# arnaucube/babyjubjub-rs

Measured on AMD Instinct MI355X. Metric: BabyJubJub fixed-base scalar mults/sec, 1048576-item batch per GPU, higher is better.
Workload: dtype u32; 1 GPU; 1M fixed-base scalar mults (generator B8), BASELINE configs[1]; batch_per_gpu=1048576, global_batch=1048576, window_bits=28, table_bytes=154618823808, streams=2, kernel=bjj_k_mul_fixed_base_2x256, resident_batches=4, library_default_window_bits=23, parallelism=independent shards, one process per GPU, no data-path collective

## Files before the change

babyjubjub-rs_amd/csrc/curve.hpp:

```cpp
#pragma once
#include "fr.hpp"

namespace bjj {

struct Consts {
  Fr A, D;
  Fr F;
  Fr FINV_PLAIN;
  Fr FINV;
  Fr L_R1, L_R2;
  Fr DP, D2P, DPINV;
  Fr B8X, B8Y;
  Fr TS_G;
  Fr HALFQ;
  Fr ORDER, ORDER2, ORDER4;
  Fr L, L2, L4;
  Fr PCF[48];
  Fr PKP[60];
  Fr PSP[660];
  Fr PAL[25];
  Fr PM[36];
  Fr PCAB[30];
  Fr TSN[384];
  Fr TSH[448];
  unsigned char TSHASH[2048];
};
#define BJJ_CONSTS_INIT                                                                                                            \
  { BJJ_K_A, BJJ_K_D, BJJ_K_F, BJJ_K_FINV_PLAIN, BJJ_K_FINV, BJJ_K_L_R1, BJJ_K_L_R2, BJJ_K_DP, BJJ_K_D2P, BJJ_K_DPINV, BJJ_K_B8X,   \
    BJJ_K_B8Y, BJJ_K_TS_G, BJJ_K_HALFQ, BJJ_K_ORDER, BJJ_K_ORDER2, BJJ_K_ORDER4, BJJ_K_L, BJJ_K_L2, BJJ_K_L4, BJJ_K_POSEIDON_CF,   \
    BJJ_K_POSEIDON_KP, BJJ_K_POSEIDON_SP, BJJ_K_POSEIDON_AL, BJJ_K_POSEIDON_M, BJJ_K_POSEIDON_CAB, BJJ_K_TS_NEG, BJJ_K_TS_HALF,    \
    BJJ_K_TS_HASH }

struct Ext { Fr X, Y, Z, T; };
struct Niels { Fr ymx, ypx, t2d; };
struct PNiels { Fr ymx, ypx, t2d, z2; };
struct RefProj { Fr x, y, z; };

BJJ_HD Ext ext_identity() {
  Ext e; e.X = fr_zero(); e.Y = fr_one(); e.Z = fr_one(); e.T = fr_zero(); return e;
}


template <bool NEED_T = true>
BJJ_HD Ext ext_madd(const Ext& p, const Niels& q) {
  Fr a = fr_mul(fr_sub_lazy(p.Y, p.X), q.ymx);
  Fr b = fr_mul(fr_add_lazy(p.Y, p.X), q.ypx);
  Fr c = fr_mul(p.T, q.t2d);
  Fr d = fr_add_lazy(p.Z, p.Z);
  Fr e = fr_sub_lazy(b, a);
  Fr f = fr_sub(d, c);
  Fr g = fr_add_lazy(d, c);
  Fr h = fr_add_lazy(b, a);
  Ext r;
  r.X = fr_mul(e, f); r.Y = fr_mul(g, h); r.Z = fr_mul(f, g);
  if (NEED_T) r.T = fr_mul(e, h); else r.T = fr_zero();
  return r;
}
struct MaddState { Fr ym, yp, d, T; };
template <bool NEED_T = true>
BJJ_HD Ext ext_madd_state(const MaddState& s, const Niels& q, bool flip = false) {
  Fr a = fr_mul(s.ym, q.ymx);
  Fr b = fr_mul(s.yp, q.ypx);
  Fr c = fr_mul(s.T, q.t2d);
  Fr h = fr_add_lazy(b, a);
  Fr e;
#pragma unroll
  for (int i = 0; i < NL; i++) {
    const u32 x = flip ? a.v[i] : b.v[i];
    BJJ_ASSERT(h.v[i] - x <= fr_c4limb(i));
    e.v[i] = (x << 1) + fr_c4limb(i) - h.v[i];
  }
  Fr f = fr_sub(s.d, c);
  Fr g = fr_add_lazy(s.d, c);
  Ext r;
  r.X = fr_mul(e, f); r.Y = fr_mul(g, h); r.Z = fr_mul(f, g);
  if (NEED_T) r.T = fr_mul(e, h); else r.T = fr_zero();
  return r;
}
BJJ_HD MaddState ext_madd_forms(const Ext& p) {
  MaddState s;
  s.ym = fr_sub_lazy(p.Y, p.X); s.yp = fr_add_lazy(p.Y, p.X); s.d = fr_add_lazy(p.Z, p.Z); s.T = p.T;
  return s;
}
BJJ_HD MaddState niels_tform_state(const Niels& e0, bool neg, bool neg_t) {
  MaddState s;
  const Fr ymx = fr_select(neg, e0.ypx, e0.ymx), ypx = fr_select(neg, e0.ymx, e0.ypx);
  s.ym = fr_add_lazy(ymx, ymx);
  s.yp = fr_add_lazy(ypx, ypx);
  s.d = fr_add(fr_add(fr_one(), fr_one()), fr_add(fr_one(), fr_one()));
  s.T = fr_select(neg_t, fr_sub_lazy(fr_zero(), e0.t2d), e0.t2d);
  return s;
}
BJJ_HD Ext ext_add_pn(const Ext& p, const PNiels& q, bool need_t = true) {
  Fr a = fr_mul(fr_sub_lazy(p.Y, p.X), q.ymx);
  Fr b = fr_mul(fr_add_lazy(p.Y, p.X), q.ypx);
  Fr c = fr_mul(p.T, q.t2d);
  Fr d = fr_mul(p.Z, q.z2);
  Fr e = fr_sub_lazy(b, a);
  Fr f = fr_sub(d, c);
  Fr g = fr_add_lazy(d, c);
  Fr h = fr_add_lazy(b, a);
  Ext r;
  r.X = fr_mul(e, f); r.Y = fr_mul(g, h); r.Z = fr_mul(f, g);
  r.T = fr_zero();
  if (need_t) r.T = fr_mul(e, h);
  return r;
}
template <bool NEED_T>
BJJ_HD Ext ext_dbl(const Ext& p) {
  Fr a = fr_sqr(p.X), b = fr_sqr(p.Y), zz = fr_sqr(p.Z);
  Fr h = fr_add_lazy(a, b);
  Fr s = fr_sqr(fr_add_lazy(p.X, p.Y));
  Fr e = fr_sub8_of_lazy(s, h);
  Fr g = fr_sub_lazy(b, a);
  Fr f = fr_sub(fr_add_lazy(fr_add_lazy(zz, zz), a), b);
  Ext r;
  r.X = fr_mul(e, f); r.Y = fr_mul(g, h); r.Z = fr_mul(f, g);
  if (NEED_T) r.T = fr_mul(e, h); else r.T = fr_zero();
  return r;
}
BJJ_HD PNiels ext_to_pniels(const Ext& p, const Consts& K) {
  PNiels n;
  n.ymx = fr_sub(p.Y, p.X); n.ypx = fr_add(p.Y, p.X);
  n.t2d = fr_mul(p.T, K.D2P); n.z2 = fr_dbl(p.Z);
  return n;
}
BJJ_HD PNiels pniels_cneg(const PNiels& n, bool neg) {
  PNiels r;
  r.ymx = fr_select(neg, n.ypx, n.ymx);
  r.ypx = fr_select(neg, n.ymx, n.ypx);
  r.t2d = fr_select(neg, fr_sub_lazy(fr_zero(), n.t2d), n.t2d);
  r.z2 = n.z2;
  return r;
}
BJJ_HD Ext ext_from_ref_affine(const Fr& x, const Fr& y, const Consts& K) {
  Ext e;
  e.X = fr_mul(x, K.F); e.Y = y; e.Z = fr_one(); e.T = fr_mul(e.X, y);
  return e;
}
BJJ_HD bool ref_on_curve(const Fr& x, const Fr& y, const Consts& K) {
  Fr x2 = fr_sqr(x), y2 = fr_sqr(y);
  Fr lhs = fr_add(fr_mul(K.A, x2), y2);
  Fr rhs = fr_add(fr_one(), fr_mul(K.D, fr_mul(x2, y2)));
  return fr_eq(lhs, rhs);
}

BJJ_HD RefProj ref_add(const RefProj& p, const RefProj& q, const Consts& K) {
  Fr a = fr_mul(p.z, q.z);
  Fr b = fr_sqr(a);
  Fr c = fr_mul(p.x, q.x);
  Fr d = fr_mul(p.y, q.y);
  Fr e = fr_mul(fr_mul(K.D, c), d);
  Fr f = fr_sub(b, e);
  Fr g = fr_add(b, e);
  Fr aux = fr_mul(fr_add(p.x, p.y), fr_add(q.x, q.y));
  aux = fr_sub(fr_sub(aux, c), d);
  Fr x3 = fr_mul(fr_mul(a, f), aux);
  Fr dac = fr_sub(d, fr_mul(K.A, c));
  Fr y3 = fr_mul(fr_mul(a, g), dac);
  RefProj r; r.x = x3; r.y = y3; r.z = fr_mul(f, g);
  return r;
}

BJJ_HD void scalar_mod_order(const u32 w[8], u32 out[8], const Consts& K) {
  Fr s = fr_from_words(w);
  s = fr_cond_sub_kr(s, K.ORDER4.v);
  s = fr_cond_sub_kr(s, K.ORDER2.v);
  s = fr_cond_sub_kr(s, K.ORDER.v);
  fr_to_words(s, out);
}
BJJ_HD Fr plain_mod_l(const Fr& v, const Consts& K) {
  Fr s = fr_cond_sub_kr(v, K.L4.v);
  s = fr_cond_sub_kr(s, K.L2.v);
  s = fr_cond_sub_kr(s, K.L.v);
  return s;
}
BJJ_HD u32 scalar_window(const u32 w[8], int j, int W) {
  const int bit = j * W, wi = bit >> 5, sh = bit & 31;
  if (wi >= 8) return 0;
  u64 two = (u64)w[wi] | ((u64)(wi + 1 < 8 ? w[wi + 1] : 0u) << 32);
  return (u32)(two >> sh) & ((1u << W) - 1u);
}

}
```

babyjubjub-rs_amd/csrc/fr.hpp:

```cpp
#pragma once
#include <stdint.h>

#if defined(__HIPCC__)
#define BJJ_HD __host__ __device__ __forceinline__
#define BJJ_HD_NOINLINE static __host__ __device__ __noinline__
#else
#define BJJ_HD inline
#define BJJ_HD_NOINLINE
#endif

#if defined(BJJ_DEBUG_BOUNDS) && !defined(__HIP_DEVICE_COMPILE__)
#include <assert.h>
#define BJJ_ASSERT(x) assert(x)
#else
#define BJJ_ASSERT(x) ((void)0)
#endif

namespace bjj {

typedef uint32_t u32;
typedef uint64_t u64;

constexpr int NL = 9;
constexpr u32 MASK29 = 0x1fffffffu;

struct Fr { u32 v[NL]; };

#define BJJ_N0 0x10000001u
#define BJJ_N1 0x1f0fac9fu
#define BJJ_N2 0x0e5c2450u
#define BJJ_N3 0x07d090f3u
#define BJJ_N4 0x1585d283u
#define BJJ_N5 0x02db40c0u
#define BJJ_N6 0x00a6e141u
#define BJJ_N7 0x0e5c2634u
#define BJJ_N8 0x0030644eu
#define BJJ_NINV29 0x0fffffffu

BJJ_HD u32 fr_modlimb(int i) {
  constexpr u32 N[NL] = {BJJ_N0, BJJ_N1, BJJ_N2, BJJ_N3, BJJ_N4, BJJ_N5, BJJ_N6, BJJ_N7, BJJ_N8};
  return N[i];
}

BJJ_HD u32 fr_c4limb(int i) {
  constexpr u32 C[NL] = {0x4u + 0x20000000u, 0x1c3eb27eu + 0x1fffffffu, 0x19709143u + 0x1fffffffu,
                         0x1f4243cdu + 0x1fffffffu, 0x16174a0cu + 0x1fffffffu, 0x0b6d0302u + 0x1fffffffu,
                         0x029b8504u + 0x1fffffffu, 0x197098d0u + 0x1fffffffu, 0x00c19139u - 1u};
  return C[i];
}
BJJ_HD u32 fr_c8limb(int i) {
  constexpr u32 C[NL] = {0x8u + 0x20000000u, 0x187d64fcu + 0x1fffffffu, 0x12e12287u + 0x1fffffffu,
                         0x1e84879bu + 0x1fffffffu, 0x0c2e9419u + 0x1fffffffu, 0x16da0605u + 0x1fffffffu,
                         0x05370a08u + 0x1fffffffu, 0x12e131a0u + 0x1fffffffu, 0x01832273u - 1u};
  return C[i];
}

BJJ_HD Fr fr_zero() { Fr r; for (int i = 0; i < NL; i++) r.v[i] = 0; return r; }

BJJ_HD void fr_carry(Fr& a) {
#pragma unroll
  for (int i = 0; i < NL - 1; i++) {
    a.v[i + 1] += a.v[i] >> 29;
    a.v[i] &= MASK29;
  }
}

BJJ_HD Fr fr_add(const Fr& a, const Fr& b) {
  Fr r;
#pragma unroll
  for (int i = 0; i < NL; i++) r.v[i] = a.v[i] + b.v[i];
  fr_carry(r);
  return r;
}
BJJ_HD Fr fr_sub(const Fr& a, const Fr& b) {
  Fr r;
  BJJ_ASSERT(b.v[8] <= fr_c4limb(8));
#pragma unroll
  for (int i = 0; i < NL; i++) r.v[i] = a.v[i] + fr_c4limb(i) - b.v[i];
  fr_carry(r);
  return r;
}
BJJ_HD Fr fr_sub8(const Fr& a, const Fr& b) {
  Fr r;
  BJJ_ASSERT(b.v[8] <= fr_c8limb(8));
#pragma unroll
  for (int i = 0; i < NL; i++) r.v[i] = a.v[i] + fr_c8limb(i) - b.v[i];
  fr_carry(r);
  return r;
}
BJJ_HD Fr fr_add_lazy(const Fr& a, const Fr& b) {
  Fr r;
#pragma unroll
  for (int i = 0; i < NL; i++) r.v[i] = a.v[i] + b.v[i];
  return r;
}
BJJ_HD Fr fr_sub_lazy(const Fr& a, const Fr& b) {
  Fr r;
  BJJ_ASSERT(b.v[8] <= fr_c4limb(8));
#pragma unroll
  for (int i = 0; i < NL; i++) { BJJ_ASSERT(b.v[i] <= fr_c4limb(i)); r.v[i] = a.v[i] + fr_c4limb(i) - b.v[i]; }
  return r;
}
BJJ_HD u32 fr_k8limb(int i) {
  constexpr u32 C[NL] = {0x8u + 0x40000000u, 0x187d64fcu + 0x3ffffffeu, 0x12e12287u + 0x3ffffffeu,
                         0x1e84879bu + 0x3ffffffeu, 0x0c2e9419u + 0x3ffffffeu, 0x16da0605u + 0x3ffffffeu,
                         0x05370a08u + 0x3ffffffeu, 0x12e131a0u + 0x3ffffffeu, 0x01832273u - 2u};
  return C[i];
}
BJJ_HD Fr fr_sub8_of_lazy(const Fr& a, const Fr& b) {
  Fr r;
#pragma unroll
  for (int i = 0; i < NL; i++) { BJJ_ASSERT(b.v[i] <= fr_k8limb(i)); r.v[i] = a.v[i] + fr_k8limb(i) - b.v[i]; }
  fr_carry(r);
  return r;
}
BJJ_HD Fr fr_neg(const Fr& a) { return fr_sub(fr_zero(), a); }
BJJ_HD Fr fr_dbl(const Fr& a) { return fr_add(a, a); }

BJJ_HD Fr fr_select(bool c, const Fr& a, const Fr& b) {
  Fr r;
#pragma unroll
  for (int i = 0; i < NL; i++) r.v[i] = c ? a.v[i] : b.v[i];
  return r;
}

#if defined(BJJ_DEBUG_BOUNDS) && !defined(__HIP_DEVICE_COMPILE__)
inline void fr_check_mul_operands(const Fr& a, const Fr& b) {
  for (int k = 0; k < 2 * NL - 1; k++) {
    unsigned __int128 col = 0;
    for (int i = 0; i < NL; i++) { int j = k - i; if (j >= 0 && j < NL) col += (unsigned __int128)a.v[i] * b.v[j]; }
    col += (unsigned __int128)9 * 0x1fffffffULL * 0x1fffffffULL + ((unsigned __int128)1 << 36);
    assert((col >> 64) == 0);
  }
  unsigned __int128 ah = (((unsigned __int128)a.v[8] << 29) + a.v[7]) + 1;
  unsigned __int128 bh = (((unsigned __int128)b.v[8] << 29) + b.v[7]) + 1;
  const unsigned __int128 lim = (((unsigned __int128)0x30644e72e131ULL << 64) | 0xa029b85045b68181ULL) >> 1;
  assert(ah * bh <= lim);
}
#define BJJ_CHECK_MUL(a, b) fr_check_mul_operands(a, b)
#else
#define BJJ_CHECK_MUL(a, b) ((void)0)
#endif

#define BJJ_MAD(acc, x, y) acc += (u64)(x) * (y)
#define BJJ_MAD_K(acc, x, k) acc += (u64)(x) * (k)

#if defined(__HIP_DEVICE_COMPILE__) && !defined(BJJ_NO_ASM_COLUMNS)
#include "fr_mul_columns.inc"
#endif

BJJ_HD Fr fr_mul(const Fr& a, const Fr& b) {
  BJJ_CHECK_MUL(a, b);
#if defined(__HIP_DEVICE_COMPILE__) && !defined(BJJ_NO_ASM_COLUMNS)
  return fr_mul_columns(a, b);
#endif
  u32 m[NL];
  Fr r;
  u64 acc = 0;
#pragma unroll
  for (int k = 0; k < NL; k++) {
#pragma unroll
    for (int i = 0; i <= k; i++) BJJ_MAD(acc, a.v[i], b.v[k - i]);
#pragma unroll
    for (int i = 0; i < k; i++) BJJ_MAD_K(acc, m[i], fr_modlimb(k - i));
    m[k] = ((u32)acc * BJJ_NINV29) & MASK29;
    BJJ_MAD_K(acc, m[k], BJJ_N0);
    acc >>= 29;
  }
#pragma unroll
  for (int k = NL; k < 2 * NL - 1; k++) {
#pragma unroll
    for (int i = k - (NL - 1); i < NL; i++) BJJ_MAD(acc, a.v[i], b.v[k - i]);
#pragma unroll
    for (int i = k - (NL - 1); i < NL; i++) BJJ_MAD_K(acc, m[i], fr_modlimb(k - i));
    r.v[k - NL] = (u32)acc & MASK29;
    acc >>= 29;
  }
  r.v[NL - 1] = (u32)acc;
  return r;
}

BJJ_HD Fr fr_sqr(const Fr& a) {
  BJJ_CHECK_MUL(a, a);
#if defined(__HIP_DEVICE_COMPILE__) && !defined(BJJ_NO_ASM_COLUMNS)
  return fr_sqr_columns(a);
#endif
  u32 m[NL], a2[NL];
#pragma unroll
  for (int i = 0; i < NL; i++) a2[i] = a.v[i] << 1;
  Fr r;
  u64 acc = 0;
#pragma unroll
  for (int k = 0; k < NL; k++) {
#pragma unroll
    for (int i = 0; 2 * i < k; i++) BJJ_MAD(acc, a2[i], a.v[k - i]);
    if ((k & 1) == 0) BJJ_MAD(acc, a.v[k / 2], a.v[k / 2]);
#pragma unroll
    for (int i = 0; i < k; i++) BJJ_MAD_K(acc, m[i], fr_modlimb(k - i));
    m[k] = ((u32)acc * BJJ_NINV29) & MASK29;
    BJJ_MAD_K(acc, m[k], BJJ_N0);
    acc >>= 29;
  }
#pragma unroll
  for (int k = NL; k < 2 * NL - 1; k++) {
#pragma unroll
    for (int i = k - (NL - 1); 2 * i < k; i++) BJJ_MAD(acc, a2[i], a.v[k - i]);
    if ((k & 1) == 0) BJJ_MAD(acc, a.v[k / 2], a.v[k / 2]);
#pragma unroll
    for (int i = k - (NL - 1); i < NL; i++) BJJ_MAD_K(acc, m[i], fr_modlimb(k - i));
    r.v[k - NL] = (u32)acc & MASK29;
    acc >>= 29;
  }
  r.v[NL - 1] = (u32)acc;
  return r;
}

BJJ_HD Fr fr_reduce_weak(const Fr& x) {
  const u32 q = x.v[8] / 3171407u;
  Fr r;
  int64_t c = 0;
#pragma unroll
  for (int i = 0; i < NL; i++) {
    c += (int64_t)x.v[i] - (int64_t)((u64)q * fr_modlimb(i));
    r.v[i] = (i < NL - 1) ? ((u32)c & MASK29) : (u32)c;
    c >>= 29;
  }
  return r;
}

BJJ_HD Fr fr_one() {
  Fr r = {{0x0fffff57u, 0x1ea70ab4u, 0x052c068bu, 0x17504f49u, 0x0aa8075bu, 0x1d4240ceu, 0x11d54c07u, 0x052ac7a8u, 0x000dc836u}};
  return r;
}
BJJ_HD Fr fr_r2() {
  Fr r = {{0x05b69bd4u, 0x06170a5au, 0x020cddceu, 0x1db6310bu, 0x0e54d0ffu, 0x1cf855e3u, 0x1c15e103u, 0x07d09161u, 0x000a054au}};
  return r;
}
BJJ_HD Fr fr_one_plain() { Fr r = fr_zero(); r.v[0] = 1; return r; }

BJJ_HD Fr fr_from_words(const u32 w[8]) {
  Fr r;
  r.v[0] = w[0] & MASK29;
#pragma unroll
  for (int i = 1; i < 8; i++) {
    const int bit = 29 * i, wi = bit >> 5, sh = bit & 31;
    u64 two = (u64)w[wi] | ((u64)(wi + 1 < 8 ? w[wi + 1] : 0u) << 32);
    r.v[i] = (u32)(two >> sh) & MASK29;
  }
  r.v[8] = w[7] >> 8;
  return r;
}
BJJ_HD void fr_to_words(const Fr& a, u32 w[8]) {
#pragma unroll
  for (int j = 0; j < 8; j++) {
    const int bit = 32 * j, li = bit / 29, sh = bit - 29 * li;
    u64 acc = (u64)a.v[li] >> sh;
    int have = 29 - sh;
    acc |= (u64)a.v[li + 1] << have;
    have += 29;
    if (have < 32 && li + 2 < NL) acc |= (u64)a.v[li + 2] << have;
    w[j] = (u32)acc;
  }
}

BJJ_HD Fr fr_cond_sub_kr(const Fr& x, const u32 kr[NL]) {
  Fr d;
  u32 borrow = 0;
#pragma unroll
  for (int i = 0; i < NL; i++) {
    u32 t = x.v[i] - kr[i] - borrow;
    borrow = t >> 31;
    d.v[i] = (i < NL - 1) ? (t & MASK29) : t;
  }
  return fr_select(borrow != 0, x, d);
}
BJJ_HD Fr fr_canon(const Fr& x) {
  constexpr u32 R8[NL] = {0x8u, 0x187d64fcu, 0x12e12287u, 0x1e84879bu, 0x0c2e9419u, 0x16da0605u, 0x05370a08u, 0x12e131a0u, 0x01832273u};
  constexpr u32 R4[NL] = {0x4u, 0x1c3eb27eu, 0x19709143u, 0x1f4243cdu, 0x16174a0cu, 0x0b6d0302u, 0x029b8504u, 0x197098d0u, 0x00c19139u};
  constexpr u32 R2[NL] = {0x2u, 0x1e1f593fu, 0x1cb848a1u, 0x0fa121e6u, 0x0b0ba506u, 0x05b68181u, 0x014dc282u, 0x1cb84c68u, 0x0060c89cu};
  constexpr u32 R1[NL] = {BJJ_N0, BJJ_N1, BJJ_N2, BJJ_N3, BJJ_N4, BJJ_N5, BJJ_N6, BJJ_N7, BJJ_N8};
  Fr t = fr_cond_sub_kr(x, R8);
  t = fr_cond_sub_kr(t, R4);
  t = fr_cond_sub_kr(t, R2);
  t = fr_cond_sub_kr(t, R1);
  return t;
}
BJJ_HD bool fr_is_zero_canon(const Fr& a) {
  u32 o = 0;
#pragma unroll
  for (int i = 0; i < NL; i++) o |= a.v[i];
  return o == 0;
}
BJJ_HD bool fr_is_zero(const Fr& a) { return fr_is_zero_canon(fr_canon(a)); }
BJJ_HD bool fr_eq(const Fr& a, const Fr& b) { return fr_is_zero(fr_sub(a, b)); }

BJJ_HD Fr fr_to_mont_words(const u32 w[8]) { return fr_mul(fr_from_words(w), fr_r2()); }
BJJ_HD void fr_from_mont_words(const Fr& a, u32 w[8]) {
  constexpr u32 R1[NL] = {BJJ_N0, BJJ_N1, BJJ_N2, BJJ_N3, BJJ_N4, BJJ_N5, BJJ_N6, BJJ_N7, BJJ_N8};
  Fr t = fr_mul(a, fr_one_plain());
  t = fr_cond_sub_kr(t, R1);
  fr_to_words(t, w);
}

BJJ_HD_NOINLINE Fr fr_inv_fermat(const Fr& a) {
  const u32 E[8] = {0xefffffffu, 0x43e1f593u, 0x79b97091u, 0x2833e848u, 0x8181585du, 0xb85045b6u, 0xe131a029u, 0x30644e72u};
  Fr x = a;
  for (int bit = 252; bit >= 0; bit--) {
    x = fr_sqr(x);
    if ((E[bit >> 5] >> (bit & 31)) & 1) x = fr_mul(x, a);
  }
  return x;
}

BJJ_HD_NOINLINE Fr fr_inv_gcd(const Fr& x) {
  constexpr u32 R32[NL] = {0x20u, 0x01f593f0u, 0x0b848a1fu, 0x1a121e6eu, 0x10ba5067u, 0x1b681815u, 0x14dc2822u, 0x0b84c680u, 0x060c89ceu};
  constexpr u32 R16[NL] = {0x10u, 0x10fac9f8u, 0x05c2450fu, 0x1d090f37u, 0x185d2833u, 0x0db40c0au, 0x0a6e1411u, 0x05c26340u, 0x030644e7u};
  constexpr u32 R8[NL] = {0x8u, 0x187d64fcu, 0x12e12287u, 0x1e84879bu, 0x0c2e9419u, 0x16da0605u, 0x05370a08u, 0x12e131a0u, 0x01832273u};
  constexpr u32 R4[NL] = {0x4u, 0x1c3eb27eu, 0x19709143u, 0x1f4243cdu, 0x16174a0cu, 0x0b6d0302u, 0x029b8504u, 0x197098d0u, 0x00c19139u};
  constexpr u32 R2c[NL] = {0x2u, 0x1e1f593fu, 0x1cb848a1u, 0x0fa121e6u, 0x0b0ba506u, 0x05b68181u, 0x014dc282u, 0x1cb84c68u, 0x0060c89cu};
  constexpr u32 R1[NL] = {BJJ_N0, BJJ_N1, BJJ_N2, BJJ_N3, BJJ_N4, BJJ_N5, BJJ_N6, BJJ_N7, BJJ_N8};
  Fr a = fr_canon(x);
  Fr b, u = fr_r2(), v = fr_zero();
#pragma unroll
  for (int i = 0; i < NL; i++) b.v[i] = fr_modlimb(i);
#pragma unroll 1
  for (int outer = 0; outer < 18; outer++) {
    u32 ah = 0, al = 0, all_ = 0, bh = 0, bl = 0, bll = 0;
    int top = 0;
#pragma unroll
    for (int i = NL - 1; i >= 2; i--) {
      const bool hit = (top == 0) && ((a.v[i] | b.v[i]) != 0);
      ah = hit ? a.v[i] : ah; al = hit ? a.v[i - 1] : al; all_ = hit ? a.v[i - 2] : all_;
      bh = hit ? b.v[i] : bh; bl = hit ? b.v[i - 1] : bl; bll = hit ? b.v[i - 2] : bll;
      top = hit ? i : top;
    }
    const int L = (top == 0) ? 0 : 32 - __builtin_clz(ah | bh);
    const bool big = 29 * top + L > 60, l2 = L >= 2;
    const int sh = l2 ? L - 2 : 0;
    const u64 ha = ((u64)ah << 29) | al, hb = ((u64)bh << 29) | bl;
    const u64 ta_s = ha >> sh, tb_s = hb >> sh;
    const u64 ta_l = (ha << 1) | (all_ >> 28), tb_l = (hb << 1) | (bll >> 28);
    const u64 ta = l2 ? ta_s : ta_l, tb = l2 ? tb_s : tb_l;
    const u64 xa_big = (ta << 29) | a.v[0], xb_big = (tb << 29) | b.v[0];
    const u64 xa_small = ((u64)a.v[2] << 58) | ((u64)a.v[1] << 29) | a.v[0];
    const u64 xb_small = ((u64)b.v[2] << 58) | ((u64)b.v[1] << 29) | b.v[0];
    u64 xa = big ? xa_big : xa_small, xb = big ? xb_big : xb_small;
    int32_t f0 = 1, g0 = 0, f1 = 0, g1 = 1;
#pragma unroll 1
    for (int i = 0; i < 29; i++) {
      const bool odd = (xa & 1) != 0;
// ... 144 lines not shown
```

babyjubjub-rs_amd/csrc/k_fixed.hip:

```cpp
#include "k_common.hpp"

#ifndef BJJ_K1_BLOCK
#define BJJ_K1_BLOCK BJJ_EPI_BLOCK
#endif
#ifndef BJJ_K1_MIN_BLOCKS
#define BJJ_K1_MIN_BLOCKS 1
#endif
#ifndef BJJ_K1_NBUF
#define BJJ_K1_NBUF 2
#endif
#ifndef BJJ_K1_INV_CORE
#define BJJ_K1_INV_CORE INV_K1
#endif
#ifndef BJJ_K1_PIPE_ITEM
#define BJJ_K1_PIPE_ITEM 1
#endif
#ifndef BJJ_K1_PIPE_RECORD
#define BJJ_K1_PIPE_RECORD 0
#endif
#ifndef BJJ_K1_EARLY_RECORD
#define BJJ_K1_EARLY_RECORD 0
#endif
#ifndef BJJ_K1_LATE_SCALAR
#define BJJ_K1_LATE_SCALAR 1
#endif
#ifndef BJJ_K1_FOLD_LIFT
#define BJJ_K1_FOLD_LIFT 1
#endif
#ifndef BJJ_K1_WEAK_MOD_L
#define BJJ_K1_WEAK_MOD_L 1
#endif
#ifndef BJJ_K1_SLOT_STRIP
#define BJJ_K1_SLOT_STRIP 1
#endif
#ifndef BJJ_K1_SIGN_CARRY
#define BJJ_K1_SIGN_CARRY 1
#endif
#ifndef BJJ_K1_REG_RECORDS
#define BJJ_K1_REG_RECORDS 1
#endif
#ifndef BJJ_K1_UNIFORM_STAGE
#define BJJ_K1_UNIFORM_STAGE 1
#endif
#ifndef BJJ_K1_ALIGN_DIGITS
#define BJJ_K1_ALIGN_DIGITS 1
#endif
#define K1_SIGN_CARRY (BJJ_K1_SIGN_CARRY && BJJ_K1_FOLD_LIFT)

__global__ void __launch_bounds__(64) bjj_k_fixed_window_bases(u32* bases, int W, int nwin) {
  const int j = blockIdx.x * blockDim.x + threadIdx.x;
  if (j >= nwin) return;
  store_niels(bases + (size_t)j * NIELS_WORDS, fixed_table_entry(1u, j, W, c_K));
}
__global__ void __launch_bounds__(BJJ_BLOCK) bjj_k_build_fixed_table(u32* table, const u32* __restrict__ bases, int W, int nwin,
                                                                 u32 chain) {
  const size_t stride = fixed_stride(W);
  const size_t cpw = (stride + chain - 1) / chain;
  const size_t t = (size_t)blockIdx.x * blockDim.x + threadIdx.x;
  if (t >= cpw * (size_t)nwin) return;
  const int j = (int)(t / cpw);
  const size_t k0 = (t % cpw) * chain;
  const u32 cnt = (u32)(stride - k0 < chain ? stride - k0 : chain);
  fixed_table_chain(table, load_niels(bases + (size_t)j * NIELS_WORDS), (size_t)j * stride + k0, (u32)k0, cnt, W, c_K);
}
__global__ void __launch_bounds__(BJJ_BLOCK) bjj_k_check_fixed_table(const u32* __restrict__ table, const u32* __restrict__ bases,
                                                                 int W, int nwin, unsigned long long* bad) {
  const size_t stride = fixed_stride(W);
  const size_t total = stride * (size_t)nwin, nthreads = (size_t)gridDim.x * blockDim.x;
  unsigned long long mine = 0;
#pragma unroll 1
  for (size_t e = (size_t)blockIdx.x * blockDim.x + threadIdx.x; e < total; e += nthreads)
    mine += (unsigned long long)fixed_table_check_slot(table, bases, (int)(e / stride), (u32)(e % stride), W, nwin, c_K);
  if (mine) atomicAdd(bad, mine);
}


struct K1Item {
  DigitStream ds;
  bool neg0, neg1;
};
__device__ __forceinline__ u32 k1_limb(u32 lo, u32 hi, int sh) { return ((lo >> sh) | (hi << (32 - sh))) & MASK29; }
__device__ __forceinline__ Fr k1_scalar_limbs(const U4 (&v)[2]) {
  Fr s;
  s.v[0] = v[0].x & MASK29;
  s.v[1] = k1_limb(v[0].x, v[0].y, 29); s.v[2] = k1_limb(v[0].y, v[0].z, 26); s.v[3] = k1_limb(v[0].z, v[0].w, 23);
  s.v[4] = k1_limb(v[0].w, v[1].x, 20); s.v[5] = k1_limb(v[1].x, v[1].y, 17); s.v[6] = k1_limb(v[1].y, v[1].z, 14);
  s.v[7] = k1_limb(v[1].z, v[1].w, 11);
  s.v[8] = v[1].w >> 8;
  return s;
}
__device__ __forceinline__ size_t k1_digit_next(DigitStream& d, bool& neg) {
  if (!BJJ_K1_ALIGN_DIGITS) return digit_next(d, neg);
  const u32 u = (d.w[0] & d.mask) + d.carry;
  neg = u > d.half;
  d.carry = neg ? 1u : 0u;
  const u32 dig = neg ? (d.mask + 1u) - u : u;
  const size_t slot = d.base + dig;
  d.base += d.stride;
#pragma unroll
  for (int i = 0; i < 7; i++) d.w[i] = __builtin_amdgcn_alignbit(d.w[i + 1], d.w[i], (u32)d.W);
  d.w[7] >>= d.W;
  return slot;
}
template <class G>
__device__ __forceinline__ K1Item k1_item_begin(const G& g, int W, const U4 (&scalar)[2]) {
  u32 sc[8];
  Fr s = scalar_mod_l_weak_limbs(k1_scalar_limbs(scalar), scalar[1].w >> 24, c_K);
  if (!BJJ_K1_WEAK_MOD_L) s = fr_cond_sub_kr(s, c_K.L.v);
  fr_to_words(s, sc);
  K1Item it;
  it.ds = digit_stream(sc, W);
  typename G::Pending p;
  g.issue(k1_digit_next(it.ds, it.neg0), p, 0);
  g.issue(k1_digit_next(it.ds, it.neg1), p, 1);
  return it;
}
#if BJJ_K1_FOLD_LIFT
typedef MaddState K1Acc;
template <bool NEED_T = true>
__device__ __forceinline__ Ext k1_madd(const K1Acc& s, const Niels& q, bool flip = false) {
  return ext_madd_state<NEED_T>(s, q, K1_SIGN_CARRY && flip);
}
__device__ __forceinline__ K1Acc k1_forms(const Ext& p) { return ext_madd_forms(p); }
#else
typedef Ext K1Acc;
template <bool NEED_T = true>
__device__ __forceinline__ Ext k1_madd(const K1Acc& s, const Niels& q, bool = false) { return ext_madd<NEED_T>(s, q); }
__device__ __forceinline__ K1Acc k1_forms(const Ext& p) { return p; }
#endif
__device__ __forceinline__ Niels k1_entry(const Niels& e, bool neg) { return K1_SIGN_CARRY ? e : niels_cneg_lazy(e, neg); }
template <class G, class MID>
__device__ __forceinline__ void k1_item_windows(const G& g, int nwin, K1Item& it, K1Acc& acc, Niels& cur, const MID& mid) {
  typename G::Pending p;
  bool neg, last = false;
#if K1_SIGN_CARRY
  acc = niels_tform_state(g.finish(p, 0), it.neg0 != it.neg1, it.neg0 != it.neg1);
  BJJ_SCHED_FENCE();
  cur = g.finish(p, 1);
  last = it.neg1;
#elif BJJ_K1_FOLD_LIFT
  const Niels e0 = g.finish(p, 0);
  const Fr ymx0 = fr_select(it.neg0, e0.ypx, e0.ymx), ypx0 = fr_select(it.neg0, e0.ymx, e0.ypx);
  acc.ym = fr_add_lazy(ymx0, ymx0);
  acc.yp = fr_add_lazy(ypx0, ypx0);
  acc.d = fr_add(fr_add(fr_one(), fr_one()), fr_add(fr_one(), fr_one()));
  acc.T = e0.t2d;
  BJJ_SCHED_FENCE();
  const Niels e1 = g.finish(p, 1);
  cur = niels_cneg_lazy(e1, it.neg1);
  cur.t2d = fr_select(it.neg0 != it.neg1, fr_sub_lazy(fr_zero(), e1.t2d), e1.t2d);
#else
  const Niels n0 = niels_cneg_lazy(g.finish(p, 0), it.neg0);
  acc.X = fr_reduce_weak(fr_sub(n0.ypx, n0.ymx));
  acc.Y = fr_add(n0.ypx, n0.ymx);
  acc.Z = fr_add(fr_one(), fr_one()); acc.T = fr_add(n0.t2d, fr_zero());
  BJJ_SCHED_FENCE();
  cur = niels_cneg_lazy(g.finish(p, 1), it.neg1);
#endif
  mid();
#pragma unroll 1
  for (int j = 1; j + 1 < nwin; j++) {
    g.issue(k1_digit_next(it.ds, neg), p, (j + 1) & 1);
    acc = k1_forms(k1_madd(acc, cur, neg != last));
    if (K1_SIGN_CARRY) last = neg;
    BJJ_SCHED_FENCE();
    cur = k1_entry(g.finish(p, (j + 1) & 1), neg);
  }
}
struct K1Stash { U4 x[2], y[2], z[2], p[2]; };
__device__ __forceinline__ void k1_words(U4 (&v)[2], const Fr& f) {
  const u32* a = f.v;
  v[0] = U4{a[0] | (a[1] << 29), (a[1] >> 3) | (a[2] << 26), (a[2] >> 6) | (a[3] << 23), (a[3] >> 9) | (a[4] << 20)};
  v[1] = U4{(a[4] >> 12) | (a[5] << 17), (a[5] >> 15) | (a[6] << 14), (a[6] >> 18) | (a[7] << 11), (a[7] >> 21) | (a[8] << 8)};
}
__device__ __forceinline__ void k1_stash_words(U4 (&v)[2], const Fr& f) {
  if (BJJ_K1_REG_RECORDS) { k1_words(v, f); return; }
  u32 w[8];
  fr_to_words(f, w);
  v[0] = U4{w[0], w[1], w[2], w[3]}; v[1] = U4{w[4], w[5], w[6], w[7]};
}
__device__ __forceinline__ void k1_stash_pack(K1Stash& s, const Ext& p, Fr& run) {
  k1_stash_words(s.x, p.X); k1_stash_words(s.y, p.Y); k1_stash_words(s.z, p.Z); k1_stash_words(s.p, run);
  run = fr_mul(run, p.Z);
}
__device__ __forceinline__ void k1_stash_store(const K1Stash& s, uint8_t* xy_item, u32* scr_item) {
  U4 *q = (U4*)xy_item, *r = (U4*)scr_item;
  q[0] = s.x[0]; q[1] = s.x[1]; q[2] = s.y[0]; q[3] = s.y[1];
  r[0] = s.z[0]; r[1] = s.z[1]; r[2] = s.p[0]; r[3] = s.p[1];
}
struct K1Record {
  U4 z[2], p[2], x[2], y[2];
};
__device__ __forceinline__ void k1_record_load(K1Record& r, const uint8_t* xy_item, const u32* scr_item) {
  const U4 *s = (const U4*)scr_item, *q = (const U4*)xy_item;
  r.z[0] = s[0]; r.z[1] = s[1]; r.p[0] = s[2]; r.p[1] = s[3];
  r.x[0] = q[0]; r.x[1] = q[1]; r.y[0] = q[2]; r.y[1] = q[3];
}
__device__ __forceinline__ Fr k1_record_fr(const U4 (&v)[2]) {
  if (BJJ_K1_REG_RECORDS) return k1_scalar_limbs(v);
  const u32 w[8] = {v[0].x, v[0].y, v[0].z, v[0].w, v[1].x, v[1].y, v[1].z, v[1].w};
  return fr_from_words(w);
}
template <unsigned FORM>
__device__ __forceinline__ void k1_record_finish(Fr& inv, uint8_t* out_item, const K1Record& r) {
  constexpr u32 R1[NL] = {BJJ_N0, BJJ_N1, BJJ_N2, BJJ_N3, BJJ_N4, BJJ_N5, BJJ_N6, BJJ_N7, BJJ_N8};
  const Fr Z = k1_record_fr(r.z), P = k1_record_fr(r.p), X = k1_record_fr(r.x), Y = k1_record_fr(r.y);
  Fr zinv = fr_mul(inv, P);
  inv = fr_mul(inv, Z);
  Fr c2 = fr_mul(zinv, c_K.FINV);
  Fr x = fr_cond_sub_kr(fr_mul(X, c2), R1);
  Fr y = fr_cond_sub_kr(fr_mul(Y, zinv), R1);
  if (BJJ_K1_REG_RECORDS) {
    U4 *const o = (U4*)out_item, v[2];
    if (FORM & EPI_COMPRESS) {
      k1_words(v, y);
      if (plain_gt_halfq(x, c_K)) v[1].w |= 0x80000000u;
      o[0] = v[0]; o[1] = v[1];
    } else {
      k1_words(v, x); o[0] = v[0]; o[1] = v[1];
      k1_words(v, y); o[2] = v[0]; o[3] = v[1];
    }
    return;
  }
  u32 w[8];
  if (FORM & EPI_COMPRESS) {
    fr_to_words(y, w);
    if (plain_gt_halfq(x, c_K)) w[7] |= 0x80000000u;
    store_w8(out_item, w);
  } else {
    fr_to_words(x, w); store_w8(out_item, w);
    fr_to_words(y, w); store_w8(out_item + 32, w);
  }
}
template <int BLOCK, unsigned FORM>
__device__ __forceinline__ void k1_epilogue_run(Fr run, size_t n, size_t tid, size_t nthreads, uint8_t* out, const uint8_t* stash,
                                                const u32* scratch, u32* lds) {
  constexpr size_t OUT_BYTES = (FORM & EPI_COMPRESS) ? 32 : 64;
  const size_t cnt = tid < n ? (n - tid + nthreads - 1) / nthreads : 0;
  K1Record cur;
  if (BJJ_K1_EARLY_RECORD && cnt) {
    asm volatile("s_waitcnt vmcnt(0)" ::: "memory");
    const size_t i = tid + (cnt - 1) * nthreads;
    k1_record_load(cur, stash + i * 64, scratch + i * 16);
  }
  Fr inv = fr_mul(block_invert<BLOCK, BJJ_K1_INV_CORE>(run, lds), fr_one_plain());
  if (!cnt) return;
  if (!BJJ_K1_EARLY_RECORD) {
    const size_t i = tid + (cnt - 1) * nthreads;
    k1_record_load(cur, stash + i * 64, scratch + i * 16);
  }
#pragma unroll 1
  for (size_t m = cnt; m-- > 0;) {
    const size_t i = tid + m * nthreads;
    if (BJJ_K1_PIPE_RECORD) {
      K1Record nxt = cur;
      if (m) k1_record_load(nxt, stash + (i - nthreads) * 64, scratch + (i - nthreads) * 16);
      k1_record_finish<FORM>(inv, out + i * OUT_BYTES, cur);
      cur = nxt;
    } else {
      k1_record_finish<FORM>(inv, out + i * OUT_BYTES, cur);
      if (m) k1_record_load(cur, stash + (i - nthreads) * 64, scratch + (i - nthreads) * 16);
    }
  }
}

template <int BLOCK, int NBUF, unsigned FORM = EPI_AFFINE, bool AHEAD = false>
__device__ __forceinline__ void mul_fixed_base_body(const u32* __restrict__ table, int W, int nwin, const uint8_t* __restrict__ scalars,
                                                    size_t n, uint8_t* __restrict__ out, u32* __restrict__ scratch,
                                                    uint8_t* __restrict__ xy = nullptr) {
  __shared__ u32 lds[NL * 64];
  constexpr bool STRIP = AHEAD && BJJ_K1_PIPE_ITEM && BJJ_K1_SLOT_STRIP;
  constexpr int WAVE_WORDS = NBUF * FB_STAGE_WORDS + (STRIP ? FB_STRIP_WORDS : 0);
  __shared__ __attribute__((aligned(16))) u32 stage[(BLOCK / 64) * WAVE_WORDS];
  const size_t tid = (size_t)blockIdx.x * blockDim.x + threadIdx.x;
  const size_t nthreads = (size_t)gridDim.x * blockDim.x;
  const int lane = threadIdx.x & 63;
  const int wave = AHEAD && BJJ_K1_UNIFORM_STAGE ? __builtin_amdgcn_readfirstlane((int)(threadIdx.x >> 6)) : (int)(threadIdx.x >> 6);
  const GatherCoopLds<NBUF, STRIP> fb = {table, stage + wave * WAVE_WORDS, lane};
  uint8_t* const stash = (FORM & EPI_COMPRESS) ? xy : out;
  Fr run = fr_one();
  if (AHEAD && BJJ_K1_PIPE_ITEM) {
    static_assert(!AHEAD || NBUF >= 2, "both gathers of the next item are issued at once");
    size_t i = tid;
    if (i - lane < n) {
      const U4* const sc4 = (const U4*)scalars;
      U4 raw[2] = {sc4[2 * (i < n ? i : n - 1)], sc4[2 * (i < n ? i : n - 1) + 1]};
      K1Item it = k1_item_begin(fb, W, raw);
      K1Stash held = {};
      bool pending = false;
      size_t iheld = 0;
#pragma unroll 1
      for (;;) {
        const size_t inext = i + nthreads, iload = inext < n ? inext : n - 1;
        const bool more = inext - lane < n;
        if (!BJJ_K1_LATE_SCALAR && more) { raw[0] = sc4[2 * iload]; raw[1] = sc4[2 * iload + 1]; }
        K1Acc acc;
        Niels cur;
        k1_item_windows(fb, nwin, it, acc, cur, [&]() {
          if (!BJJ_K1_LATE_SCALAR) return;
          if (pending) k1_stash_store(held, stash + iheld * 64, scratch + iheld * 16);
          if (more) { raw[0] = sc4[2 * iload]; raw[1] = sc4[2 * iload + 1]; }
        });
        if (more) it = k1_item_begin(fb, W, raw);
        BJJ_SCHED_FENCE();
        const Ext p = k1_madd<false>(acc, cur);
        pending = BJJ_K1_LATE_SCALAR && more;
        if (pending) { k1_stash_pack(held, p, run); iheld = i; }
        else if (i < n) {
          if (BJJ_K1_REG_RECORDS) { k1_stash_pack(held, p, run); k1_stash_store(held, stash + i * 64, scratch + i * 16); }
          else epilogue_stash(p, run, stash + i * 64, scratch + i * 16);
        }
        if (!more) break;
        i = inext;
      }
    }
  } else {
#pragma unroll 1
    for (size_t i = tid; i - lane < n; i += nthreads) {
      const bool valid = i < n;
      u32 sc[8];
      load_w8(scalars + (valid ? i : n - 1) * 32, sc);
      Ext p = fixed_base_mul(fb, W, nwin, sc, c_K);
      if (valid) epilogue_stash(p, run, stash + i * 64, scratch + i * 16);
    }
  }
  if (AHEAD && (BJJ_K1_REG_RECORDS || BJJ_K1_PIPE_RECORD || BJJ_K1_EARLY_RECORD))
    k1_epilogue_run<BLOCK, FORM>(run, n, tid, nthreads, out, stash, scratch, lds);
  else
    epilogue_run<BLOCK, FORM, BJJ_K1_INV_CORE>(run, n, tid, nthreads, out, scratch, lds, xy);
}
__global__ void __launch_bounds__(BJJ_K1_BLOCK, BJJ_K1_MIN_BLOCKS) bjj_k_mul_fixed_base(const u32* __restrict__ table, int W, int nwin,
                                                                  const uint8_t* __restrict__ scalars, size_t n,
                                                                  uint8_t* __restrict__ out, u32* __restrict__ scratch) {
  mul_fixed_base_body<BJJ_K1_BLOCK, BJJ_K1_NBUF>(table, W, nwin, scalars, n, out, scratch);
}
template <unsigned FORM>
__device__ __forceinline__ void mul_fixed_base_scan_body(const u32* __restrict__ table, int W, const uint8_t* __restrict__ scalars, size_t n,
                                                         uint8_t* __restrict__ out, u32* __restrict__ scratch, uint8_t* __restrict__ xy, int nwin) {
  __shared__ u32 lds[NL * 64];
  const size_t tid = (size_t)blockIdx.x * blockDim.x + threadIdx.x;
  const size_t nthreads = (size_t)gridDim.x * blockDim.x;
  const GatherScan fb = {table, (u32)fixed_stride(W)};
  Fr run = fr_one();
#pragma unroll 1
  for (size_t i = tid; i < n; i += nthreads) {
    u32 sc[8];
    load_w8(scalars + i * 32, sc);
    Ext p = fixed_base_mul(fb, W, nwin, sc, c_K);
    epilogue_stash(p, run, ((FORM & EPI_COMPRESS) ? xy : out) + i * 64, scratch + i * 16);
  }
  epilogue_run<BJJ_EPI_BLOCK, FORM, BJJ_K1_INV_CORE>(run, n, tid, nthreads, out, scratch, lds, xy);
}
__global__ void __launch_bounds__(BJJ_EPI_BLOCK, 1) bjj_k_mul_fixed_base_scan(const u32* __restrict__ table, int W, int nwin,
                                                                        const uint8_t* __restrict__ scalars, size_t n,
                                                                        uint8_t* __restrict__ out, u32* __restrict__ scratch) {
  mul_fixed_base_scan_body<EPI_AFFINE>(table, W, scalars, n, out, scratch, nullptr, nwin);
}
__global__ void __launch_bounds__(256, 2) bjj_k_mul_fixed_base_2x256(const u32* __restrict__ table, int W, int nwin,
                                                                    const uint8_t* __restrict__ scalars, size_t n,
                                                                    uint8_t* __restrict__ out, u32* __restrict__ scratch) {
  mul_fixed_base_body<256, 2, EPI_AFFINE, true>(table, W, nwin, scalars, n, out, scratch);
}
__global__ void __launch_bounds__(BJJ_K1_BLOCK, BJJ_K1_MIN_BLOCKS) bjj_k_mul_fixed_base_c32(const u32* __restrict__ table, int W, int nwin,
                                                                      const uint8_t* __restrict__ scalars, size_t n,
                                                                      uint8_t* __restrict__ out32, u32* __restrict__ scratch,
                                                                      uint8_t* __restrict__ xy) {
  mul_fixed_base_body<BJJ_K1_BLOCK, BJJ_K1_NBUF, EPI_COMPRESS>(table, W, nwin, scalars, n, out32, scratch, xy);
}
__global__ void __launch_bounds__(256, 2) bjj_k_mul_fixed_base_2x256_c32(const u32* __restrict__ table, int W, int nwin,
                                                                        const uint8_t* __restrict__ scalars, size_t n,
                                                                        uint8_t* __restrict__ out32, u32* __restrict__ scratch,
                                                                        uint8_t* __restrict__ xy) {
  mul_fixed_base_body<256, 2, EPI_COMPRESS, true>(table, W, nwin, scalars, n, out32, scratch, xy);
}
__global__ void __launch_bounds__(BJJ_EPI_BLOCK, 1) bjj_k_mul_fixed_base_scan_c32(const u32* __restrict__ table, int W, int nwin,
                                                                            const uint8_t* __restrict__ scalars, size_t n,
                                                                            uint8_t* __restrict__ out32, u32* __restrict__ scratch,
                                                                            uint8_t* __restrict__ xy) {
  mul_fixed_base_scan_body<EPI_COMPRESS>(table, W, scalars, n, out32, scratch, xy, nwin);
}

namespace bjjk {
int fixed_base_lanes_per_cu(int variant) {
  return variant ? lanes_for_both(bjj_k_mul_fixed_base_2x256, bjj_k_mul_fixed_base_2x256_c32, 256)
                 : lanes_for_both(bjj_k_mul_fixed_base, bjj_k_mul_fixed_base_c32, BJJ_K1_BLOCK);
}
hipError_t fill_fixed_table(hipStream_t st, u32* table, const u32* bases, int W, int nwin) {
  const size_t entries = fixed_stride(W) * (size_t)nwin;
  size_t chain = entries >> 18;
  chain = chain < 4 ? 4 : (chain > 256 ? 256 : chain);
  const size_t chains = ((fixed_stride(W) + chain - 1) / chain) * (size_t)nwin;
  BJJ_LAUNCH(bjj_k_build_fixed_table, dim3((unsigned)((chains + BJJ_BLOCK - 1) / BJJ_BLOCK)), dim3(BJJ_BLOCK), 0, st,
                     table, bases, W, nwin, (u32)chain);
  return hipGetLastError();
}
hipError_t build_fixed_table(hipStream_t st, u32* table, u32* bases, int W, int nwin) {
  BJJ_LAUNCH(bjj_k_fixed_window_bases, dim3((nwin + 63) / 64), dim3(64), 0, st, bases, W, nwin);
  return fill_fixed_table(st, table, bases, W, nwin);
}
hipError_t check_fixed_table(hipStream_t st, int grid, const u32* table, const u32* bases, int W, int nwin,
                             unsigned long long* d_bad) {
  BJJ_LAUNCH(bjj_k_check_fixed_table, dim3((unsigned)grid), dim3(BJJ_BLOCK), 0, st, table, bases, W, nwin, d_bad);
  return hipGetLastError();
}
hipError_t mul_fixed_base_scan(hipStream_t st, int cus, const u32* table, int W, int nwin, const uint8_t* scalars, size_t n,
                               uint8_t* out, u32* scratch, uint8_t* xy) {
  const int occ = xy ? occupancy_of(bjj_k_mul_fixed_base_scan_c32, BJJ_EPI_BLOCK) : occupancy_of(bjj_k_mul_fixed_base_scan, BJJ_EPI_BLOCK);
  const int grid = capped_grid(n, BJJ_EPI_BLOCK, (size_t)cus * (size_t)occ);
  if (xy)
    BJJ_LAUNCH(bjj_k_mul_fixed_base_scan_c32, dim3(grid), dim3(BJJ_EPI_BLOCK), 0, st, table, W, nwin, scalars, n, out, scratch, xy);
  else
    BJJ_LAUNCH(bjj_k_mul_fixed_base_scan, dim3(grid), dim3(BJJ_EPI_BLOCK), 0, st, table, W, nwin, scalars, n, out, scratch);
  return hipGetLastError();
}
hipError_t mul_fixed_base(hipStream_t st, int cus, int lanes_per_cu, int variant, const u32* table, int W, int nwin, const uint8_t* scalars,
                          size_t n, uint8_t* out, u32* scratch, uint8_t* xy) {
  const int block = variant ? 256 : BJJ_K1_BLOCK;
  const int grid = capped_grid(n, block, (size_t)cus * (size_t)(lanes_per_cu / block));
  if (xy) {
    if (variant)
      BJJ_LAUNCH(bjj_k_mul_fixed_base_2x256_c32, dim3(grid), dim3(256), 0, st, table, W, nwin, scalars, n, out, scratch, xy);
    else
      BJJ_LAUNCH(bjj_k_mul_fixed_base_c32, dim3(grid), dim3(BJJ_K1_BLOCK), 0, st, table, W, nwin, scalars, n, out, scratch, xy);
  } else if (variant)
    BJJ_LAUNCH(bjj_k_mul_fixed_base_2x256, dim3(grid), dim3(256), 0, st, table, W, nwin, scalars, n, out, scratch);
  else
    BJJ_LAUNCH(bjj_k_mul_fixed_base, dim3(grid), dim3(BJJ_K1_BLOCK), 0, st, table, W, nwin, scalars, n, out, scratch);
  return hipGetLastError();
}
}
```

Measured before the change: 2.044 billion scalar mults/s.

## Fold final madd into affine normalization using split G/F batch-inversion products

Instead of forming the full extended point X=ef, Y=gh, Z=fg after the last mixed addition, the kernel keeps e,h,f,g and stashes e·(prefix of g), h·(prefix of f), g and f. Two separate running products over g and f are kept and inverted together, so affine x=e/g and y=h/f come out directly. This removes the Z=fg multiply and restructures the per-item epilogue multiplies, but adds a second running product and extra per-item multiplies in the inverse-propagation pass.

Measured after the change: 2.063 billion scalar mults/s, median of 6. No clear change (+0.9%).

```diff
diff --git a/babyjubjub-rs_amd/csrc/curve.hpp b/babyjubjub-rs_amd/csrc/curve.hpp
--- a/babyjubjub-rs_amd/csrc/curve.hpp
+++ b/babyjubjub-rs_amd/csrc/curve.hpp
@@ -77,6 +77,22 @@
   if (NEED_T) r.T = fr_mul(e, h); else r.T = fr_zero();
   return r;
 }
+struct MaddTail { Fr e, h, f, g; };
+BJJ_HD MaddTail ext_madd_tail(const Fr& a, const Fr& b, const Fr& c, const Fr& d) {
+  MaddTail r;
+  r.h = fr_add_lazy(b, a);
+  r.e = fr_sub_lazy(b, a);
+  r.g = fr_add(d, c);
+  BJJ_ASSERT(c.v[8] <= fr_c2limb(8));
+#pragma unroll
+  for (int i = 0; i < NL; i++) { BJJ_ASSERT(c.v[i] <= fr_c2limb(i)); r.f.v[i] = d.v[i] + fr_c2limb(i) - c.v[i]; }
+  fr_carry(r.f);
+  BJJ_ASSERT(r.g.v[8] < (1u << 24) && r.f.v[8] < (1u << 24));
+  return r;
+}
+BJJ_HD MaddTail ext_madd_tail(const MaddState& s, const Niels& q) {
+  return ext_madd_tail(fr_mul(s.ym, q.ymx), fr_mul(s.yp, q.ypx), fr_mul(s.T, q.t2d), s.d);
+}
 BJJ_HD MaddState ext_madd_forms(const Ext& p) {
   MaddState s;
   s.ym = fr_sub_lazy(p.Y, p.X); s.yp = fr_add_lazy(p.Y, p.X); s.d = fr_add_lazy(p.Z, p.Z); s.T = p.T;
diff --git a/babyjubjub-rs_amd/csrc/fr.hpp b/babyjubjub-rs_amd/csrc/fr.hpp
--- a/babyjubjub-rs_amd/csrc/fr.hpp
+++ b/babyjubjub-rs_amd/csrc/fr.hpp
@@ -46,6 +46,12 @@
   constexpr u32 C[NL] = {0x4u + 0x20000000u, 0x1c3eb27eu + 0x1fffffffu, 0x19709143u + 0x1fffffffu,
                          0x1f4243cdu + 0x1fffffffu, 0x16174a0cu + 0x1fffffffu, 0x0b6d0302u + 0x1fffffffu,
                          0x029b8504u + 0x1fffffffu, 0x197098d0u + 0x1fffffffu, 0x00c19139u - 1u};
+  return C[i];
+}
+BJJ_HD u32 fr_c2limb(int i) {
+  constexpr u32 C[NL] = {0x2u + 0x20000000u, 0x1e1f593fu + 0x1fffffffu, 0x1cb848a1u + 0x1fffffffu,
+                         0x0fa121e6u + 0x1fffffffu, 0x0b0ba506u + 0x1fffffffu, 0x05b68181u + 0x1fffffffu,
+                         0x014dc282u + 0x1fffffffu, 0x1cb84c68u + 0x1fffffffu, 0x0060c89cu - 1u};
   return C[i];
 }
 BJJ_HD u32 fr_c8limb(int i) {
diff --git a/babyjubjub-rs_amd/csrc/k_fixed.hip b/babyjubjub-rs_amd/csrc/k_fixed.hip
--- a/babyjubjub-rs_amd/csrc/k_fixed.hip
+++ b/babyjubjub-rs_amd/csrc/k_fixed.hip
@@ -46,6 +46,10 @@
 #define BJJ_K1_ALIGN_DIGITS 1
 #endif
 #define K1_SIGN_CARRY (BJJ_K1_SIGN_CARRY && BJJ_K1_FOLD_LIFT)
+#ifndef BJJ_K1_AFFINE_TAIL
+#define BJJ_K1_AFFINE_TAIL 1
+#endif
+#define K1_AFFINE_TAIL (BJJ_K1_AFFINE_TAIL && BJJ_K1_FOLD_LIFT && BJJ_K1_REG_RECORDS && BJJ_K1_PIPE_ITEM)
 
 __global__ void __launch_bounds__(64) bjj_k_fixed_window_bases(u32* bases, int W, int nwin) {
   const int j = blockIdx.x * blockDim.x + threadIdx.x;
@@ -183,6 +187,13 @@
   k1_stash_words(s.x, p.X); k1_stash_words(s.y, p.Y); k1_stash_words(s.z, p.Z); k1_stash_words(s.p, run);
   run = fr_mul(run, p.Z);
 }
+#if K1_AFFINE_TAIL
+__device__ __forceinline__ void k1_stash_pack(K1Stash& s, const MaddTail& t, Fr& rg, Fr& rf) {
+  k1_words(s.x, fr_mul(t.e, rg)); k1_words(s.y, fr_mul(t.h, rf)); k1_words(s.z, t.g); k1_words(s.p, t.f);
+  rg = fr_mul(rg, t.g);
+  rf = fr_mul(rf, t.f);
+}
+#endif
 __device__ __forceinline__ void k1_stash_store(const K1Stash& s, uint8_t* xy_item, u32* scr_item) {
   U4 *q = (U4*)xy_item, *r = (U4*)scr_item;
   q[0] = s.x[0]; q[1] = s.x[1]; q[2] = s.y[0]; q[3] = s.y[1];
@@ -201,6 +212,35 @@
   const u32 w[8] = {v[0].x, v[0].y, v[0].z, v[0].w, v[1].x, v[1].y, v[1].z, v[1].w};
   return fr_from_words(w);
 }
+template <unsigned FORM>
+__device__ __forceinline__ void k1_result_store(uint8_t* out_item, const Fr& x, const Fr& y) {
+  U4 *const o = (U4*)out_item, v[2];
+  if (FORM & EPI_COMPRESS) {
+    k1_words(v, y);
+    if (plain_gt_halfq(x, c_K)) v[1].w |= 0x80000000u;
+    o[0] = v[0]; o[1] = v[1];
+  } else {
+    k1_words(v, x); o[0] = v[0]; o[1] = v[1];
+    k1_words(v, y); o[2] = v[0]; o[3] = v[1];
+  }
+}
+#if K1_AFFINE_TAIL
+__device__ __forceinline__ void k1_tail_split(const Fr& winv, const Fr& rg, const Fr& rf, Fr& ig, Fr& jf) {
+  const Fr t = fr_mul(winv, fr_one_plain());
+  jf = fr_mul(t, rg);
+  ig = fr_mul(fr_mul(t, rf), c_K.FINV);
+}
+template <unsigned FORM>
+__device__ __forceinline__ void k1_record_finish(Fr& ig, Fr& jf, uint8_t* out_item, const K1Record& r) {
+  constexpr u32 R1[NL] = {BJJ_N0, BJJ_N1, BJJ_N2, BJJ_N3, BJJ_N4, BJJ_N5, BJJ_N6, BJJ_N7, BJJ_N8};
+  const Fr G = k1_record_fr(r.z), F = k1_record_fr(r.p), U = k1_record_fr(r.x), V = k1_record_fr(r.y);
+  const Fr x = fr_cond_sub_kr(fr_mul(ig, U), R1);
+  const Fr y = fr_cond_sub_kr(fr_mul(jf, V), R1);
+  ig = fr_mul(ig, G);
+  jf = fr_mul(jf, F);
+  k1_result_store<FORM>(out_item, x, y);
+}
+#endif
 template <unsigned FORM>
 __device__ __forceinline__ void k1_record_finish(Fr& inv, uint8_t* out_item, const K1Record& r) {
   constexpr u32 R1[NL] = {BJJ_N0, BJJ_N1, BJJ_N2, BJJ_N3, BJJ_N4, BJJ_N5, BJJ_N6, BJJ_N7, BJJ_N8};
@@ -210,18 +250,7 @@
   Fr c2 = fr_mul(zinv, c_K.FINV);
   Fr x = fr_cond_sub_kr(fr_mul(X, c2), R1);
   Fr y = fr_cond_sub_kr(fr_mul(Y, zinv), R1);
-  if (BJJ_K1_REG_RECORDS) {
-    U4 *const o = (U4*)out_item, v[2];
-    if (FORM & EPI_COMPRESS) {
-      k1_words(v, y);
-      if (plain_gt_halfq(x, c_K)) v[1].w |= 0x80000000u;
-      o[0] = v[0]; o[1] = v[1];
-    } else {
-      k1_words(v, x); o[0] = v[0]; o[1] = v[1];
-      k1_words(v, y); o[2] = v[0]; o[3] = v[1];
-    }
-    return;
-  }
+  if (BJJ_K1_REG_RECORDS) { k1_result_store<FORM>(out_item, x, y); return; }
   u32 w[8];
   if (FORM & EPI_COMPRESS) {
     fr_to_words(y, w);
@@ -233,7 +262,7 @@
   }
 }
 template <int BLOCK, unsigned FORM>
-__device__ __forceinline__ void k1_epilogue_run(Fr run, size_t n, size_t tid, size_t nthreads, uint8_t* out, const uint8_t* stash,
+__device__ __forceinline__ void k1_epilogue_run(Fr run, Fr run2, size_t n, size_t tid, size_t nthreads, uint8_t* out, const uint8_t* stash,
                                                 const u32* scratch, u32* lds) {
   constexpr size_t OUT_BYTES = (FORM & EPI_COMPRESS) ? 32 : 64;
   const size_t cnt = tid < n ? (n - tid + nthreads - 1) / nthreads : 0;
@@ -243,7 +272,14 @@
     const size_t i = tid + (cnt - 1) * nthreads;
     k1_record_load(cur, stash + i * 64, scratch + i * 16);
   }
+#if K1_AFFINE_TAIL
+  Fr inv, inv2;
+  k1_tail_split(block_invert<BLOCK, BJJ_K1_INV_CORE>(fr_mul(run, run2), lds), run, run2, inv, inv2);
+#define K1_FINISH(i) k1_record_finish<FORM>(inv, inv2, out + (i) * OUT_BYTES, cur)
+#else
   Fr inv = fr_mul(block_invert<BLOCK, BJJ_K1_INV_CORE>(run, lds), fr_one_plain());
+#define K1_FINISH(i) k1_record_finish<FORM>(inv, out + (i) * OUT_BYTES, cur)
+#endif
   if (!cnt) return;
   if (!BJJ_K1_EARLY_RECORD) {
     const size_t i = tid + (cnt - 1) * nthreads;
@@ -255,13 +291,14 @@
     if (BJJ_K1_PIPE_RECORD) {
       K1Record nxt = cur;
       if (m) k1_record_load(nxt, stash + (i - nthreads) * 64, scratch + (i - nthreads) * 16);
-      k1_record_finish<FORM>(inv, out + i * OUT_BYTES, cur);
+      K1_FINISH(i);
       cur = nxt;
     } else {
-      k1_record_finish<FORM>(inv, out + i * OUT_BYTES, cur);
+      K1_FINISH(i);
       if (m) k1_record_load(cur, stash + (i - nthreads) * 64, scratch + (i - nthreads) * 16);
     }
   }
+#undef K1_FINISH
 }
 
 template <int BLOCK, int NBUF, unsigned FORM = EPI_AFFINE, bool AHEAD = false>
@@ -278,7 +315,7 @@
   const int wave = AHEAD && BJJ_K1_UNIFORM_STAGE ? __builtin_amdgcn_readfirstlane((int)(threadIdx.x >> 6)) : (int)(threadIdx.x >> 6);
   const GatherCoopLds<NBUF, STRIP> fb = {table, stage + wave * WAVE_WORDS, lane};
   uint8_t* const stash = (FORM & EPI_COMPRESS) ? xy : out;
-  Fr run = fr_one();
+  Fr run = fr_one(), run2 = fr_one();
   if (AHEAD && BJJ_K1_PIPE_ITEM) {
     static_assert(!AHEAD || NBUF >= 2, "both gathers of the next item are issued at once");
     size_t i = tid;
@@ -303,13 +340,20 @@
         });
         if (more) it = k1_item_begin(fb, W, raw);
         BJJ_SCHED_FENCE();
+        pending = BJJ_K1_LATE_SCALAR && more;
+#if K1_AFFINE_TAIL
+        const MaddTail p = ext_madd_tail(acc, cur);
+        if (pending || i < n) k1_stash_pack(held, p, run, run2);
+        if (pending) iheld = i;
+        else if (i < n) k1_stash_store(held, stash + i * 64, scratch + i * 16);
+#else
         const Ext p = k1_madd<false>(acc, cur);
-        pending = BJJ_K1_LATE_SCALAR && more;
         if (pending) { k1_stash_pack(held, p, run); iheld = i; }
         else if (i < n) {
           if (BJJ_K1_REG_RECORDS) { k1_stash_pack(held, p, run); k1_stash_store(held, stash + i * 64, scratch + i * 16); }
           else epilogue_stash(p, run, stash + i * 64, scratch + i * 16);
         }
+#endif
         if (!more) break;
         i = inext;
       }
@@ -325,7 +369,7 @@
     }
   }
   if (AHEAD && (BJJ_K1_REG_RECORDS || BJJ_K1_PIPE_RECORD || BJJ_K1_EARLY_RECORD))
-    k1_epilogue_run<BLOCK, FORM>(run, n, tid, nthreads, out, stash, scratch, lds);
+    k1_epilogue_run<BLOCK, FORM>(run, run2, n, tid, nthreads, out, stash, scratch, lds);
   else
     epilogue_run<BLOCK, FORM, BJJ_K1_INV_CORE>(run, n, tid, nthreads, out, scratch, lds, xy);
 }
```
